# fuxiao0719/PanopticNeRF

Hardware: AMD Instinct MI355X
Metric: Msamples/sec (coarse+fine), KITTI-360 1408x376 (higher is better)
Workload: dtype bf16

## Files before the change

panopticnerf_amd/csrc/pnr_composite.hip:

```cpp
#include "pnr_composite_dev.h"

struct CompositeArgs {
    const float* raw; int64_t stride_s, stride_c;
    const float* z; const float* rays; const float* noise;
    const int32_t* label_sem; const int32_t* label_inst;
    int64_t R; int N, C, K, sem_mode, white_bkgd;
    float *rgb, *depth, *acc, *weights, *sem, *inst, *fix_sem, *fix_inst;
    int use_hist;
};

#ifndef CMP_GRID_PER_CU
#define CMP_GRID_PER_CU 8
#endif
#ifndef CMP_UB
#define CMP_UB 8
#endif

__device__ __forceinline__ float dot4(const f4& w, const f4& v)
{
    return fmaf(w.v[3], v.v[3], fmaf(w.v[2], v.v[2], fmaf(w.v[1], v.v[1], w.v[0] * v.v[0])));
}

template <bool CH_MAJOR, int SUB, bool SOFTMAX, class... Rng>
__global__ __launch_bounds__(256) void k_composite(CompositeArgs a, const Rng... rng)
{
    constexpr bool RNG = sizeof...(Rng) > 0;
    extern __shared__ __attribute__((aligned(16))) uint32_t s_hist[];
    RayLanes<SUB, 1> rl(a.R);
    const int wave = threadIdx.x >> 6;
    const int N = a.N, q = rl.q;
    const int CK = a.C + a.K;
    const int nq = 3 + CK;
    uint32_t* hist = s_hist + ((size_t)wave * rl.RPW + rl.g) * CK;
    PnrRngKey key;
    if constexpr (RNG) key = pnr_rng_key(rng...);

    const int64_t first = ((int64_t)blockIdx.x * blockDim.x + threadIdx.x) >> 6;
    const int64_t step = ((int64_t)gridDim.x * blockDim.x) >> 6;
    for (int64_t grp = first; grp < rl.n_groups; grp += step) {
        rl.at(grp, a.R, N);
        const int64_t ray = rl.ray, s0 = rl.s0;
        const bool active = rl.act[0];
        const bool writer = active && q == 0;

        const f4 zz = ld4(a.z + s0, active);
        f4 sg = load4<CH_MAJOR>(a.raw, a.stride_s, a.stride_c, s0, 3, active);
        f4 nxt[CMP_UB];
#pragma unroll
        for (int j = 0; j < CMP_UB; ++j) nxt[j] = load4<CH_MAJOR>(a.raw, a.stride_s, a.stride_c, s0, j < 3 ? j : j + 1, active && j < nq);
        add_sigma_noise4<RNG>(sg.v, active, key, (uint32_t)ray, (uint32_t)q, a.noise, a.noise + s0);
        const float dn = ray_dir_norm(a.rays, rl.rayc);
        const float znext = __shfl_down(zz.v[0], 1, 64);
        f4 alpha, Tl, w;
        float P = alpha_chain<4>(zz.v, znext, sg.v, rl.i0, N, dn, alpha.v, Tl.v);
        if (!active) P = 1.0f;
        const float excl = scan_excl_shfl<SUB>(P, q);
#pragma unroll
        for (int k = 0; k < 4; ++k) w.v[k] = active ? (alpha.v[k] * Tl.v[k]) * excl : 0.0f;
        if (a.weights) st4(a.weights + s0, w.v, active);
        const float accv = group_sum<SUB>((w.v[0] + w.v[1]) + (w.v[2] + w.v[3]));
        const float depv = group_sum<SUB>(dot4(w, zz));
        if (writer) {
            if (a.depth) a.depth[ray] = depv;
            if (a.acc) a.acc[ray] = accv;
        }

        const bool want_fs = a.fix_sem && a.label_sem && a.C, want_fi = a.fix_inst && a.label_inst && a.K;
        if (want_fs || want_fi) {
            int ls[4], li[4];
            ld4_labels(a.label_sem + s0, active && want_fs, ls);
            ld4_labels(a.label_inst + s0, active && want_fi, li);
            if (a.use_hist) {
                hist_zero<SUB>(hist, q, CK);
#pragma unroll
                for (int k = 0; k < 4; ++k) hist_add(hist, w.v[k], want_fs, ls[k], a.C, want_fi, li[k], a.K);
                if (rl.valid) hist_store<SUB>(hist, q, ray, want_fs, a.fix_sem, a.C, want_fi, a.fix_inst, a.K);
            } else {
                for (int c = 0; c < CK; ++c) {
                    const bool is_s = c < a.C;
                    if ((is_s && !want_fs) || (!is_s && !want_fi)) continue;
                    const int cc = is_s ? c : c - a.C;
                    float p = 0.0f;
#pragma unroll
                    for (int k = 0; k < 4; ++k) p += ((is_s ? ls[k] : li[k]) == cc) ? w.v[k] : 0.0f;
                    const float r = group_sum<SUB>(p);
                    if (writer) (is_s ? a.fix_sem : a.fix_inst)[ray * (is_s ? a.C : a.K) + cc] = r;
                }
            }
        }

        f4 mx_s, den_s, mx_i, den_i;
        if constexpr (SOFTMAX) {
            auto field_stats = [&](int nch, int ch0, f4& mx, f4& den) {
#pragma unroll
                for (int k = 0; k < 4; ++k) { mx.v[k] = -INFINITY; den.v[k] = 0.0f; }
                for (int c = 0; c < nch; ++c) {
                    const f4 v = load4<CH_MAJOR>(a.raw, a.stride_s, a.stride_c, s0, ch0 + c, active);
#pragma unroll
                    for (int k = 0; k < 4; ++k) lse_step(mx.v[k], den.v[k], v.v[k]);
                }
            };
            field_stats(a.C, 4, mx_s, den_s);
            field_stats(a.K, 4 + a.C, mx_i, den_i);
        }

#pragma unroll 1
        for (int q0 = 0; q0 < nq; q0 += CMP_UB) {
            float r[CMP_UB];
            const bool more = q0 + CMP_UB < nq;
#pragma unroll
            for (int j = 0; j < CMP_UB; ++j) {
                const int qq = q0 + j;
                f4 v = nxt[j];
                if (qq < 3) {
#pragma unroll
                    for (int k = 0; k < 4; ++k) v.v[k] = sigmoid_of(v.v[k]);
                } else if constexpr (SOFTMAX) {
                    const bool fs = (qq - 3) < a.C;
#pragma unroll
                    for (int k = 0; k < 4; ++k) v.v[k] = softmax_of(v.v[k], fs ? mx_s.v[k] : mx_i.v[k], fs ? den_s.v[k] : den_i.v[k]);
                }
                r[j] = dot4(w, v);
                const int q2 = qq + CMP_UB;
                if (more) nxt[j] = load4<CH_MAJOR>(a.raw, a.stride_s, a.stride_c, s0, q2 + 1, active && q2 < nq);
            }
            group_sum_batch<SUB, CMP_UB>(r);
            if (writer) store_rows<CMP_UB>(a, ray, q0, nq, r, accv);
        }
    }
}

#ifndef CMP2_UB
#define CMP2_UB 8
#endif

template <int L, int M4, bool SOFTMAX, class... Rng>
__global__ __launch_bounds__(256) void k_composite2(CompositeArgs a, const Rng... rng)
{
    constexpr bool RNG = sizeof...(Rng) > 0;
    extern __shared__ __attribute__((aligned(16))) uint32_t s_hist[];
    constexpr int M = 4 * M4;
    RayLanes<L, M4> rl(a.R);
    const int wave = threadIdx.x >> 6;
    const int N = a.N, q = rl.q, i0 = rl.i0;
    const int CK = a.C + a.K;
    const int nq = 3 + CK;
    uint32_t* hist = s_hist + ((size_t)wave * rl.RPW + rl.g) * CK;
    const int64_t sc = a.stride_c;
    PnrRngKey key;
    if constexpr (RNG) key = pnr_rng_key(rng...);

    const int64_t first = ((int64_t)blockIdx.x * blockDim.x + threadIdx.x) >> 6;
    const int64_t step = ((int64_t)gridDim.x * blockDim.x) >> 6;
    for (int64_t grp = first; grp < rl.n_groups; grp += step) {
        rl.at(grp, a.R, N);
        const int64_t ray = rl.ray, s0 = rl.s0;
        const bool (&act)[M4] = rl.act;
        const bool writer = rl.valid && q == 0;

        float zz[M], w[M];
        ld_row<M4>(a.z + s0, act, zz);
        ld_row<M4>(a.raw + 3 * sc + s0, act, w);
        float nxt[CMP2_UB][M];
#pragma unroll
        for (int j = 0; j < CMP2_UB; ++j) {
            if (j < nq) ld_row<M4>(a.raw + (int64_t)(j < 3 ? j : j + 1) * sc + s0, act, nxt[j]);
        }
#pragma unroll
        for (int j = 0; j < M4; ++j)
            add_sigma_noise4<RNG>(w + 4 * j, act[j], key, (uint32_t)ray, (uint32_t)((i0 >> 2) + j), a.noise, a.noise + s0 + 4 * j);
        const float dn = ray_dir_norm(a.rays, rl.rayc);
        const float znext = dpp_or<0x101>(zz[0], 0.0f);
        float alpha[M], Tl[M];
        float P = alpha_chain<M>(zz, znext, w, i0, N, dn, alpha, Tl);
        if (!act[0]) P = 1.0f;
        const float excl = scan_excl_dpp<L>(P, q);
        float accp = 0.0f, depp = 0.0f;
#pragma unroll
        for (int k = 0; k < M; ++k) {
            w[k] = act[k >> 2] ? (alpha[k] * Tl[k]) * excl : 0.0f;
            accp += w[k];
            depp = fmaf(w[k], zz[k], depp);
        }
        if (a.weights) {
#pragma unroll
            for (int j = 0; j < M4; ++j) st4(a.weights + s0 + 4 * j, w + 4 * j, act[j]);
        }
        const float accv = group_sum<L>(accp);
        const float depv = group_sum<L>(depp);
        if (writer) {
            if (a.depth) a.depth[ray] = depv;
            if (a.acc) a.acc[ray] = accv;
        }

        const bool want_fs = a.fix_sem && a.label_sem && a.C, want_fi = a.fix_inst && a.label_inst && a.K;
        if (want_fs || want_fi) {
            hist_zero<L>(hist, q, CK);
#pragma unroll
            for (int j = 0; j < M4; ++j) {
                int ls[4], li[4];
                ld4_labels(a.label_sem + s0 + 4 * j, act[j] && want_fs, ls);
                ld4_labels(a.label_inst + s0 + 4 * j, act[j] && want_fi, li);
#pragma unroll
                for (int k = 0; k < 4; ++k) hist_add(hist, w[4 * j + k], want_fs, ls[k], a.C, want_fi, li[k], a.K);
            }
            if (rl.valid) hist_store<L>(hist, q, ray, want_fs, a.fix_sem, a.C, want_fi, a.fix_inst, a.K);
        }

        float mx_s[SOFTMAX ? M : 1], den_s[SOFTMAX ? M : 1], mx_i[SOFTMAX ? M : 1], den_i[SOFTMAX ? M : 1];
        if constexpr (SOFTMAX) {
            auto field_stats = [&](int nch, int ch0, float (&mx)[M], float (&den)[M]) {
#pragma unroll
                for (int k = 0; k < M; ++k) { mx[k] = -INFINITY; den[k] = 0.0f; }
                for (int c = 0; c < nch; ++c) {
                    float v[M];
                    ld_row<M4>(a.raw + (int64_t)(ch0 + c) * sc + s0, act, v);
#pragma unroll
                    for (int k = 0; k < M; ++k) lse_step(mx[k], den[k], v[k]);
                }
            };
            field_stats(a.C, 4, mx_s, den_s);
            field_stats(a.K, 4 + a.C, mx_i, den_i);
        }

#pragma unroll 1
        for (int q0 = 0; q0 < nq; q0 += CMP2_UB) {
            float r[CMP2_UB];
#pragma unroll
            for (int j = 0; j < CMP2_UB; ++j) {
                const int qq = q0 + j;
                float acc = 0.0f;
#pragma unroll
                for (int k = 0; k < M; ++k) {
                    float v = nxt[j][k];
                    if (qq < 3) v = sigmoid_of(v);
                    else if constexpr (SOFTMAX) {
                        const bool fs = (qq - 3) < a.C;
                        v = softmax_of(v, fs ? mx_s[k] : mx_i[k], fs ? den_s[k] : den_i[k]);
                    }
                    acc = fmaf(w[k], v, acc);
                }
                r[j] = acc;
                const int q2 = qq + CMP2_UB;
                if (q2 < nq) ld_row<M4>(a.raw + (int64_t)(q2 + 1) * sc + s0, act, nxt[j]);
            }
            group_sum_batch<L, CMP2_UB>(r);
            if (writer) store_rows<CMP2_UB>(a, ray, q0, nq, r, accv);
        }
    }
}

static int composite_impl(const float* raw, int64_t raw_stride_s, int64_t raw_stride_c, const float* z, const float* rays,
                          const float* noise, const PnrRngDev* rng, const int32_t* label_sem, const int32_t* label_inst, int64_t n_rays,
                          int n_samples, int n_sem, int n_inst, int sem_mode, int white_bkgd, float* rgb, float* depth, float* acc,
                          float* weights, float* sem, float* inst, float* fix_sem, float* fix_inst, void* stream)
{
    PNR_REQUIRE(n_rays <= 0 || (raw && z && rays), "pnr_composite: null pointer");
    PNR_REQUIRE(n_samples >= 4 && n_samples <= 256 && (n_samples % 4) == 0,
                "pnr_composite: n_samples=%d must be a multiple of 4 in [4,256]", n_samples);
    PNR_REQUIRE(n_sem >= 0 && n_inst >= 0 && (sem_mode == 0 || sem_mode == 1), "pnr_composite: bad field sizes");
    PNR_REQUIRE((((uintptr_t)z) & 15) == 0, "pnr_composite: z must be 16-byte aligned");
    PNR_REQUIRE(!weights || (((uintptr_t)weights) & 15) == 0, "pnr_composite: weights must be 16-byte aligned");
    PNR_REQUIRE((((uintptr_t)noise) & 15) == 0 && (((uintptr_t)label_sem) & 15) == 0 && (((uintptr_t)label_inst) & 15) == 0,
                "pnr_composite: noise / label arrays must be 16-byte aligned");
    if (n_rays <= 0) return PNR_OK;
    CompositeArgs a;
    a.raw = raw; a.stride_s = raw_stride_s; a.stride_c = raw_stride_c; a.z = z; a.rays = rays; a.noise = noise;
    a.label_sem = label_sem; a.label_inst = label_inst; a.R = n_rays; a.N = n_samples; a.C = n_sem; a.K = n_inst;
    a.sem_mode = sem_mode; a.white_bkgd = white_bkgd; a.rgb = rgb; a.depth = depth; a.acc = acc; a.weights = weights;
    a.sem = sem; a.inst = inst; a.fix_sem = fix_sem; a.fix_inst = fix_inst;
    const bool want_fix = (fix_sem && label_sem && n_sem) || (fix_inst && label_inst && n_inst);
    const bool ch_major = raw_stride_s == 1 && (raw_stride_c % 4) == 0 && (((uintptr_t)raw) & 15) == 0;
    hipStream_t st = (hipStream_t)stream;
    auto hist_bytes = [&](int rpw) { return (size_t)4 * rpw * (n_sem + n_inst) * sizeof(uint32_t); };
    auto grid_for = [&](int rpw) { return pnr_grid_cap(((n_rays + rpw - 1) / rpw + 3) / 4, CMP_GRID_PER_CU); };
    if (ch_major && n_samples > 32 && n_samples <= 64 && (!want_fix || hist_bytes(8) <= 48 * 1024)) {
        a.use_hist = want_fix ? 1 : 0;
        const size_t lds = want_fix ? hist_bytes(8) : 0;
        composite_dispatch<8>(8, true, sem_mode, rng, [&](auto L, auto, auto SM, const auto&... r) {
            hipLaunchKernelGGL((k_composite2<decltype(L)::value, 2, decltype(SM)::value, std::decay_t<decltype(r)>...>), dim3(grid_for(8)), dim3(256),
                               lds, st, a, r...);
        });
        PNR_CHECK_LAUNCH("pnr_composite");
        return PNR_OK;
    }
    int sub = 1;
    while (sub < n_samples / 4) sub <<= 1;
    const int rpw = 64 / sub;
    a.use_hist = (want_fix && hist_bytes(rpw) <= 48 * 1024) ? 1 : 0;
    const size_t lds = a.use_hist ? hist_bytes(rpw) : 0;
    composite_dispatch<1, 2, 4, 8, 16, 32, 64>(sub, ch_major, sem_mode, rng, [&](auto S, auto CH, auto SM, const auto&... r) {
        hipLaunchKernelGGL((k_composite<decltype(CH)::value, decltype(S)::value, decltype(SM)::value, std::decay_t<decltype(r)>...>),
                           dim3(grid_for(rpw)), dim3(256), lds, st, a, r...);
    });
    PNR_CHECK_LAUNCH("pnr_composite");
    return PNR_OK;
}

PNR_EXPORT int pnr_composite(const float* raw, int64_t raw_stride_s, int64_t raw_stride_c, const float* z,
                             const float* rays, const float* noise, const int32_t* label_sem,
                             const int32_t* label_inst, int64_t n_rays, int n_samples, int n_sem, int n_inst,
                             int sem_mode, int white_bkgd, float* rgb, float* depth, float* acc, float* weights,
                             float* sem, float* inst, float* fix_sem, float* fix_inst, void* stream)
{
    return composite_impl(raw, raw_stride_s, raw_stride_c, z, rays, noise, nullptr, label_sem, label_inst, n_rays, n_samples, n_sem, n_inst,
                          sem_mode, white_bkgd, rgb, depth, acc, weights, sem, inst, fix_sem, fix_inst, stream);
}

PNR_EXPORT int pnr_composite_rng(const float* raw, int64_t raw_stride_s, int64_t raw_stride_c, const float* z, const float* rays,
                                 const pnr_rng* noise_host, const int32_t* label_sem, const int32_t* label_inst, int64_t n_rays,
                                 int n_samples, int n_sem, int n_inst, int sem_mode, int white_bkgd, float* rgb, float* depth, float* acc,
                                 float* weights, float* sem, float* inst, float* fix_sem, float* fix_inst, void* stream)
{
    PnrRngDev rng;
    const int rc = pnr_rng_check(noise_host, n_rays < 0 ? 0 : n_rays, "pnr_composite_rng", &rng);
    if (rc) return rc;
    PNR_REQUIRE(n_rays <= 0 || (raw_stride_s == 1 && (raw_stride_c % 4) == 0 && (((uintptr_t)raw) & 15) == 0),
                "pnr_composite_rng: channel-major, 16-byte aligned raw images only");
    return composite_impl(raw, raw_stride_s, raw_stride_c, z, rays, nullptr, &rng, label_sem, label_inst, n_rays, n_samples, n_sem, n_inst,
                          sem_mode, white_bkgd, rgb, depth, acc, weights, sem, inst, fix_sem, fix_inst, stream);
}

struct CombineArgs {
    const float* rec; int rec_floats; const float4* ps; const float* z; const int32_t* lab_s; const int32_t* lab_i;
    int64_t R; int N, C, K, white_bkgd;
    float *rgb, *depth, *acc, *weights, *sem, *inst, *fix_sem, *fix_inst;
};

template <bool LOGITS>
__global__ __launch_bounds__(256) void k_composite_combine(CombineArgs a)
{
    __shared__ uint32_t hist_all[4][128];
    const int lane = threadIdx.x & 63, wv = threadIdx.x >> 6;
    const int64_t ray = ((int64_t)blockIdx.x * blockDim.x + threadIdx.x) >> 6;
    if (ray >= a.R) return;
    const int N = a.N, T = N >> 5, RF = a.rec_floats, C = a.C, K = a.K, CK = C + K;
    const float* __restrict__ rec = a.rec + ray * T * RF;
    const float4* __restrict__ ps = a.ps + ray * N;
    const float* __restrict__ zr = a.z + ray * N;
    const bool want_s = a.lab_s && a.fix_sem && C, want_i = a.lab_i && a.fix_inst && K;
    const int32_t* __restrict__ lsr = want_s ? a.lab_s + ray * N : nullptr;
    const int32_t* __restrict__ lir = want_i ? a.lab_i + ray * N : nullptr;
    float q[8];
#pragma unroll
    for (int k = 0; k < 8; ++k) q[k] = k < T ? rec[k * RF] : 1.0f;
    float4 pv[4];
    float zv[4];
    int lsv[4], liv[4];
#pragma unroll
    for (int j = 0; j < 4; ++j) {
        const int i = lane + 64 * j;
        const bool in = i < N;
        pv[j] = in ? ps[i] : float4{0.0f, 0.0f, 0.0f, 0.0f};
        zv[j] = in ? zr[i] : 0.0f;
        lsv[j] = (in && want_s) ? lsr[i] : -1;
        liv[j] = (in && want_i) ? lir[i] : -1;
    }
    float lg[2][8];
#pragma unroll
    for (int h = 0; h < 2; ++h)
#pragma unroll
        for (int k = 0; k < 8; ++k) lg[h][k] = (LOGITS && k < T && lane + 64 * h < CK) ? rec[k * RF + PNR_FUSE_REC_LOGITS + lane + 64 * h] : 0.0f;
    float Tk[8];
    float t = 1.0f;
#pragma unroll
    for (int k = 0; k < 8; ++k) {
        Tk[k] = t;
        if (k < T) t *= q[k];
    }
    uint32_t* hist = hist_all[wv];
    if (want_s || want_i) hist_zero<64>(hist, lane, CK);
    float r5[5] = {0.0f, 0.0f, 0.0f, 0.0f, 0.0f};
#pragma unroll
    for (int j = 0; j < 4; ++j) {
        const int i = lane + 64 * j;
        if (i < N) {
            const float4 p = pv[j];
            float tk = Tk[0];
#pragma unroll
            for (int k = 1; k < 8; ++k) tk = (i >> 5) == k ? Tk[k] : tk;
            const float w = tk * p.x;
            r5[0] += w;
            r5[1] = fmaf(w, zv[j], r5[1]);
            r5[2] = fmaf(w, sigmoid_of(p.y), r5[2]);
            r5[3] = fmaf(w, sigmoid_of(p.z), r5[3]);
            r5[4] = fmaf(w, sigmoid_of(p.w), r5[4]);
            if (a.weights) a.weights[ray * N + i] = w;
            if (want_s || want_i) hist_add(hist, w, want_s, lsv[j], C, want_i, liv[j], K);
        }
    }
    group_sum_batch<64, 5>(r5);
    if (lane == 0) {
        if (a.acc) a.acc[ray] = r5[0];
        if (a.depth) a.depth[ray] = r5[1];
    }
    if (lane < 3 && a.rgb) {
        const float v = lane == 0 ? r5[2] : lane == 1 ? r5[3] : r5[4];
        a.rgb[ray * 3 + lane] = a.white_bkgd ? v + (1.0f - r5[0]) : v;
    }
#pragma unroll
    for (int h = 0; h < 2; ++h) {
        const int c = lane + 64 * h;
        if (c >= CK) continue;
        if constexpr (LOGITS) {
            float v = 0.0f;
#pragma unroll
            for (int k = 0; k < 8; ++k) if (k < T) v = fmaf(Tk[k], lg[h][k], v);
            if (c < C) { if (a.sem) a.sem[ray * C + c] = v; }
            else if (a.inst) a.inst[ray * K + (c - C)] = v;
        }
        if (c < C) { if (want_s) a.fix_sem[ray * C + c] = hist_read(hist, c); }
        else if (want_i) a.fix_inst[ray * K + (c - C)] = hist_read(hist, c);
    }
}

int pnr_composite_combine_launch(const float* rec, int rec_floats, bool logit_sums, const float4* ps, const float* z,
                                 const int32_t* label_sem, const int32_t* label_inst, int64_t R, int N, int C, int K, int white_bkgd,
                                 float* rgb, float* depth, float* acc, float* weights, float* sem, float* inst, float* fix_sem,
                                 float* fix_inst, hipStream_t st)
{
    CombineArgs a;
    a.rec = rec; a.rec_floats = rec_floats; a.ps = ps; a.z = z; a.lab_s = label_sem; a.lab_i = label_inst;
    a.R = R; a.N = N; a.C = C; a.K = K; a.white_bkgd = white_bkgd;
    a.rgb = rgb; a.depth = depth; a.acc = acc; a.weights = weights; a.sem = sem; a.inst = inst; a.fix_sem = fix_sem; a.fix_inst = fix_inst;
    const int64_t blocks = (R + 3) / 4;
    if (logit_sums) hipLaunchKernelGGL(k_composite_combine<true>, dim3((unsigned)blocks), dim3(256), 0, st, a);
    else hipLaunchKernelGGL(k_composite_combine<false>, dim3((unsigned)blocks), dim3(256), 0, st, a);
    PNR_CHECK_LAUNCH("pnr_mlp_forward_composite (combine)");
    return PNR_OK;
}
```

panopticnerf_amd/csrc/pnr_sampling.hip:

```cpp
#include "pnr_common.h"
#include "pnr_philox.h"
#include "pnr_sampling_dev.h"
#include <stdlib.h>
#include <string.h>

template <class... Rng>
__global__ __launch_bounds__(256) void k_stratified(const float* __restrict__ rays, int64_t R, int N,
                                                     int lindisp, const float* __restrict__ t_rand,
                                                     float* __restrict__ z_out, const Rng... rng)
{
    constexpr bool RNG = sizeof...(Rng) > 0;
    PnrRngKey key;
    if constexpr (RNG) key = pnr_rng_key(rng...);
    const int64_t total = R * N;
    for (int64_t s = (int64_t)blockIdx.x * blockDim.x + threadIdx.x; s < total;
         s += (int64_t)gridDim.x * blockDim.x) {
        const int64_t r = s / N;
        const int i = (int)(s - r * N);
        if constexpr (RNG) {
            const float t = pnr_rng_uniform_at(key, (uint32_t)r, i);
            z_out[s] = strat_sample(rays[r * 8 + 6], rays[r * 8 + 7], i, N, lindisp, &t);
        } else {
            z_out[s] = strat_sample(rays[r * 8 + 6], rays[r * 8 + 7], i, N, lindisp, t_rand ? t_rand + s : nullptr);
        }
    }
}

__global__ __launch_bounds__(256) void k_points(const float* __restrict__ rays, const float* __restrict__ z,
                                                 int64_t R, int N, float* __restrict__ pts)
{
    const int64_t total = R * N * 3;
    for (int64_t e = (int64_t)blockIdx.x * blockDim.x + threadIdx.x; e < total;
         e += (int64_t)gridDim.x * blockDim.x) {
        const int64_t s = e / 3;
        const int a = (int)(e - s * 3);
        const int64_t r = s / N;
        const float m = rays[r * 8 + 3 + a] * z[s];
        pts[e] = rays[r * 8 + a] + m;
    }
}

__global__ __launch_bounds__(256) void k_embed(const float* __restrict__ x, int64_t n, int L,
                                                float* __restrict__ out)
{
    const int E = 3 + 6 * L;
    const int64_t total = n * E;
    for (int64_t e = (int64_t)blockIdx.x * blockDim.x + threadIdx.x; e < total;
         e += (int64_t)gridDim.x * blockDim.x) {
        const int64_t s = e / E;
        const int c = (int)(e - s * E);
        float v;
        if (c < 3) {
            v = x[s * 3 + c];
        } else {
            const int k = (c - 3) / 6, j = (c - 3) - 6 * k;
            const int a = j % 3;
            const float arg = x[s * 3 + a] * ldexpf(1.0f, k);
            v = (j < 3) ? sinf(arg) : cosf(arg);
        }
        out[e] = v;
    }
}

struct PdfLabelArgs {
    const float* hit_t; const int32_t* hit_box; const int32_t* hit_count; int max_hits; const int32_t* box_ids;
    int32_t* label_sem; int32_t* label_inst;
};
#define PDF_MAXC 256
#define PDF_MAXT 512
template <int MAXC, int MAXT, class... Rng>
__device__ __forceinline__ void sample_pdf_body(const float* __restrict__ z, const float* __restrict__ weights,
                                                    const float* __restrict__ u, int64_t R, int Nc, int Nf,
                                                    float* __restrict__ zs_out, int32_t* __restrict__ inds_out,
                                                    float* __restrict__ zfine_out, const PdfLabelArgs lab, const Rng&... rng)
{
    constexpr bool RNG = sizeof...(Rng) > 0;
    PnrRngKey key;
    if constexpr (RNG) key = pnr_rng_key(rng...);
    __shared__ float s_z[MAXC], s_w[MAXC], s_pdf[MAXC], s_cdf[MAXC], s_bins[MAXC];
    __shared__ float s_sort[MAXT], s_out[MAXT];
    __shared__ float s_total, s_part[32];
    const int lane = threadIdx.x;
    const int nb = Nc - 1, nw = Nc - 2, Nt = Nc + Nf;
    const int P = pdf_padded(Nt);
    auto labels = [&](int64_t r, const float* sorted) {
        if (!lab.label_sem) return;
        const int mh = lab.max_hits;
        const int cnt = lab.hit_count[r] < mh ? lab.hit_count[r] : mh;
        for (int i = lane; i < Nt; i += 64) {
            const int best = label_hit(sorted[i], cnt, [&](int h, float& ti, float& to) {
                ti = lab.hit_t[(r * mh + h) * 2];
                to = lab.hit_t[(r * mh + h) * 2 + 1];
            });
            int ls, li;
            hit_ids(best, lab.hit_box + r * mh + best, lab.box_ids, &ls, &li);
            lab.label_sem[r * Nt + i] = ls;
            lab.label_inst[r * Nt + i] = li;
        }
    };
    for (int64_t r = blockIdx.x; r < R; r += gridDim.x) {
        for (int i = lane; i < Nc; i += 64) {
            s_z[i] = z[r * Nc + i];
            s_w[i] = weights[r * Nc + i];
        }
        __syncthreads();
        for (int k = lane; k < nb; k += 64) s_bins[k] = 0.5f * (s_z[k + 1] + s_z[k]);
        const float total = pdf_torch_total(s_w, nw, s_part, &s_total, lane);
        for (int j = lane; j < nw; j += 64) s_pdf[j] = (s_w[j + 1] + 1e-5f) / total;
        __syncthreads();
        pdf_cdf(lane < nw ? s_pdf[lane < nw ? lane : 0] : 0.0f, nw, nw <= 64, s_pdf, s_cdf, lane);
        for (int i = lane; i < Nf; i += 64) {
            float uu;
            if constexpr (RNG) uu = pnr_rng_uniform_at(key, (uint32_t)r, i);
            else uu = u ? u[r * Nf + i] : pnr_linspace01(i, Nf);
            int lo = 0, hi = nb;
            while (lo < hi) {
                const int mid = (lo + hi) >> 1;
                if (s_cdf[mid] <= uu) lo = mid + 1; else hi = mid;
            }
            const float zs = pdf_invert(uu, lo, nb, s_cdf, s_bins);
            if (zs_out) zs_out[r * Nf + i] = zs;
            if (inds_out) inds_out[r * Nf + i] = lo;
            s_sort[Nc + i] = zs;
        }
        if (zfine_out) {
            __syncthreads();
            bool asc = true;
            for (int i = lane; i + 1 < Nf; i += 64) asc = asc && (s_sort[Nc + i] <= s_sort[Nc + i + 1]);
            for (int i = lane; i + 1 < Nc; i += 64) asc = asc && (s_z[i] <= s_z[i + 1]);
            if (__all(asc)) {
                for (int i = lane; i < Nc; i += 64) {
                    const float v = s_z[i];
                    int lo = 0, hi = Nf;
                    while (lo < hi) { const int mid = (lo + hi) >> 1; if (s_sort[Nc + mid] < v) lo = mid + 1; else hi = mid; }
                    s_out[i + lo] = v;
                }
                for (int j = lane; j < Nf; j += 64) {
                    const float v = s_sort[Nc + j];
                    int lo = 0, hi = Nc;
                    while (lo < hi) { const int mid = (lo + hi) >> 1; if (s_z[mid] <= v) lo = mid + 1; else hi = mid; }
                    s_out[j + lo] = v;
                }
                __syncthreads();
                for (int i = lane; i < Nt; i += 64) zfine_out[r * Nt + i] = s_out[i];
                labels(r, s_out);
                __syncthreads();
                continue;
            }
            for (int i = lane; i < Nc; i += 64) s_sort[i] = s_z[i];
            for (int i = Nt + lane; i < P; i += 64) s_sort[i] = INFINITY;
            __syncthreads();
            pdf_bitonic(s_sort, P, lane);
            for (int i = lane; i < Nt; i += 64) zfine_out[r * Nt + i] = s_sort[i];
            labels(r, s_sort);
        }
        __syncthreads();
    }
}

__device__ __noinline__ void pdf_bitonic_fallback(float* s_sort, const float* s_z, const float* s_zs, int Nc, int Nf, int P, int lane)
{
    const int Nt = Nc + Nf;
    for (int i = lane; i < Nc; i += 64) s_sort[i] = s_z[i];
    for (int i = lane; i < Nf; i += 64) s_sort[Nc + i] = s_zs[i];
    for (int i = Nt + lane; i < P; i += 64) s_sort[i] = INFINITY;
    __syncthreads();
    pdf_bitonic(s_sort, P, lane);
}

#ifndef PDF_DET_WPE
#define PDF_DET_WPE 8
#endif
#if PDF_DET_WPE
__attribute__((amdgpu_waves_per_eu(PDF_DET_WPE, PDF_DET_WPE)))
#endif
__global__ __launch_bounds__(64) void k_sample_pdf_det(const float* __restrict__ z, const float* __restrict__ weights, int64_t R, int Nc,
                                                        int Nf, float* __restrict__ zfine_out, const PdfLabelArgs lab)
{
    __shared__ float s_z[64], s_w[64], s_pdf[64], s_cdf[64], s_bins[64];
    __shared__ float s_zs[192], s_out[256];
    __shared__ float s_total, s_part[32];
    const int lane = threadIdx.x;
    const int nb = Nc - 1, nw = Nc - 2, Nt = Nc + Nf;
    int topc = 1, topf = 1;
    while (topc * 2 <= Nc) topc *= 2;
    while (topf * 2 <= Nf) topf *= 2;
    const int mh = lab.max_hits;
    for (int64_t r = blockIdx.x; r < R; r += gridDim.x) {
        const float* __restrict__ zr = z + r * Nc;
        const float* __restrict__ wr = weights + r * Nc;
        const float zl = lane < Nc ? zr[lane] : 0.0f, wl = lane < Nc ? wr[lane] : 0.0f;
        int cnt = 0, h_ls = -1, h_li = -1;
        float h_ti = 0.0f, h_to = 0.0f;
        if (lab.label_sem) {
            const int c0 = lab.hit_count[r];
            cnt = c0 < mh ? c0 : mh;
            if (lane < cnt) {
                const float2 t2 = *reinterpret_cast<const float2*>(lab.hit_t + (r * mh + lane) * 2);
                h_ti = t2.x; h_to = t2.y;
                hit_ids(lane, lab.hit_box + r * mh + lane, lab.box_ids, &h_ls, &h_li);
            }
        }
        s_z[lane] = zl;
        s_w[lane] = wl;
        const float zn = __shfl_down(zl, 1, 64), wn = __shfl_down(wl, 1, 64);
        s_bins[lane] = 0.5f * (zn + zl);
        __syncthreads();
        const float total = pdf_torch_total(s_w, nw, s_part, &s_total, lane);
        const float pl = lane < nw ? (wn + 1e-5f) / total : 0.0f;
        s_pdf[lane] = pl;
        pdf_cdf(pl, nw, true, s_pdf, s_cdf, lane);
        bool asc = lane + 1 >= Nc || zl <= zn;
        for (int i = lane; i < Nf; i += 64) {
            const float uu = pnr_linspace01(i, Nf);
            int pos = 0;
            for (int st = topc; st >= 1; st >>= 1) {
                const int p = pos + st, q = p <= nb ? p : nb;
                pos = (p <= nb && s_cdf[q - 1] <= uu) ? p : pos;
            }
            s_zs[i] = pdf_invert(uu, pos, nb, s_cdf, s_bins);
        }
        __syncthreads();
        for (int i = lane; i + 1 < Nf; i += 64) asc = asc && (s_zs[i] <= s_zs[i + 1]);
        if (__all(asc)) {
            if (lane < Nc) {
                int pos = 0;
                for (int st = topf; st >= 1; st >>= 1) {
                    const int p = pos + st, q = p <= Nf ? p : Nf;
                    pos = (p <= Nf && s_zs[q - 1] < zl) ? p : pos;
                }
                s_out[lane + pos] = zl;
            }
            for (int j = lane; j < Nf; j += 64) {
                const float v = s_zs[j];
                int pos = 0;
                for (int st = topc; st >= 1; st >>= 1) {
                    const int p = pos + st, q = p <= Nc ? p : Nc;
                    pos = (p <= Nc && s_z[q - 1] <= v) ? p : pos;
                }
                s_out[j + pos] = v;
            }
            __syncthreads();
        } else {
            pdf_bitonic_fallback(s_out, s_z, s_zs, Nc, Nf, pdf_padded(Nt), lane);
        }
        float* __restrict__ zo = zfine_out + r * Nt;
        for (int i0 = 0; i0 < Nt; i0 += 256) {
            float zz[4];
            int best[4], ls[4], li[4];
            float bt[4];
#pragma unroll
            for (int k = 0; k < 4; ++k) {
                const int i = i0 + lane + 64 * k;
                zz[k] = i < Nt ? s_out[i < Nt ? i : 0] : 0.0f;
                best[k] = -1; ls[k] = -1; li[k] = -1; bt[k] = 0.0f;
                if (i < Nt) zo[i] = zz[k];
            }
            if (lab.label_sem) {
                for (int h = 0; h < cnt; ++h) {
                    const float ti = __int_as_float(__builtin_amdgcn_readlane(__float_as_int(h_ti), h));
                    const float to = __int_as_float(__builtin_amdgcn_readlane(__float_as_int(h_to), h));
                    const int hs = __builtin_amdgcn_readlane(h_ls, h), hi2 = __builtin_amdgcn_readlane(h_li, h);
#pragma unroll
                    for (int k = 0; k < 4; ++k) {
                        const bool take = ti <= zz[k] && zz[k] <= to && (best[k] < 0 || ti < bt[k]);
                        best[k] = take ? h : best[k];
                        bt[k] = take ? ti : bt[k];
                        ls[k] = take ? hs : ls[k];
                        li[k] = take ? hi2 : li[k];
                    }
                }
#pragma unroll
                for (int k = 0; k < 4; ++k) {
                    const int i = i0 + lane + 64 * k;
                    if (i < Nt) {
                        lab.label_sem[r * Nt + i] = ls[k];
                        lab.label_inst[r * Nt + i] = li[k];
                    }
                }
            }
        }
        __syncthreads();
    }
}

template <int MAXC, int MAXT, class... Rng>
__global__ __launch_bounds__(64) __attribute__((amdgpu_waves_per_eu(MAXC <= 64 ? 8 : 1, 8)))
void k_sample_pdf(const float* __restrict__ z, const float* __restrict__ weights, const float* __restrict__ u, int64_t R, int Nc, int Nf,
                  float* __restrict__ zs_out, int32_t* __restrict__ inds_out, float* __restrict__ zfine_out, const PdfLabelArgs lab,
                  const Rng... rng)
{
    sample_pdf_body<MAXC, MAXT>(z, weights, u, R, Nc, Nf, zs_out, inds_out, zfine_out, lab, rng...);
}

__global__ __launch_bounds__(256) void k_bbox_hits(const float* __restrict__ rays, int64_t R,
                                                    const float* __restrict__ box, int M, int max_hits,
                                                    float* __restrict__ hit_t, int32_t* __restrict__ hit_box,
                                                    int32_t* __restrict__ hit_count)
{
    for (int64_t r = (int64_t)blockIdx.x * blockDim.x + threadIdx.x; r < R;
         r += (int64_t)gridDim.x * blockDim.x) {
        const RayRec ry = ray_load(rays, r);
        const auto list = hit_rows(hit_t, hit_box, r, max_hits);
        hit_init(list, max_hits);
        int cnt = 0;
        for (int m = 0; m < M; ++m) {
            float tmin, tmax;
            slab_interval(box + m * 15, ry, &tmin, &tmax);
            if (tmin <= tmax) hit_insert(list, cnt, max_hits, tmin, tmax, m);
        }
        hit_count[r] = cnt;
    }
}

#define SETUP_MAXH 8
struct RaySetupArgs {
    const float* rays; int64_t R; const float* box; int M; int max_hits; const int32_t* box_ids;
    int N, lindisp, hull; const float* t_rand;
    float* hit_t; int32_t* hit_box; int32_t* hit_count; float* z; int32_t* label_sem; int32_t* label_inst;
};
template <class... Rng>
__global__ __launch_bounds__(256) void k_ray_setup(const RaySetupArgs a, const Rng... rng)
{
    constexpr bool RNG = sizeof...(Rng) > 0;
    __shared__ float2 s_t[SETUP_MAXH][64];
    __shared__ float s_nr[64], s_fr[64];
    __shared__ int s_hb[SETUP_MAXH][64], s_cnt[64];
    const int tid = threadIdx.x, lane = tid & 63, wv = tid >> 6;
    const int mh = a.max_hits, N = a.N;
    PnrRngKey key;
    if constexpr (RNG) key = pnr_rng_key(rng...);
    for (int64_t base = (int64_t)blockIdx.x * 64; base < a.R; base += (int64_t)gridDim.x * 64) {
        const int64_t r = base + tid;
        if (tid < 64 && r < a.R) {
            const float4 ra = *reinterpret_cast<const float4*>(a.rays + r * 8), rb = *reinterpret_cast<const float4*>(a.rays + r * 8 + 4);
            const float o0 = ra.x, o1 = ra.y, o2 = ra.z, d0 = ra.w, d1 = rb.x, d2 = rb.y;
            float nr = rb.z, fr = rb.w;
            for (int h = 0; h < SETUP_MAXH; ++h) { s_hb[h][tid] = -1; s_t[h][tid] = make_float2(0.0f, 0.0f); }
            int cnt = 0;
            for (int m = 0; m < a.M; ++m) {
                const float* b = a.box + m * 15;
                const float p0 = o0 - b[0], p1 = o1 - b[1], p2 = o2 - b[2];
                float tmin = nr, tmax = fr;
#pragma unroll
                for (int x = 0; x < 3; ++x) {
                    const float r0 = b[3 + 3 * x], r1 = b[4 + 3 * x], r2 = b[5 + 3 * x];
                    const float ol = (r0 * p0 + r1 * p1) + r2 * p2;
                    const float dl = (r0 * d0 + r1 * d1) + r2 * d2;
                    const float inv = 1.0f / dl;
                    const float e = b[12 + x];
                    const float t1 = (-e - ol) * inv, t2 = (e - ol) * inv;
                    tmin = fmaxf(tmin, fminf(t1, t2));
                    tmax = fminf(tmax, fmaxf(t1, t2));
                }
                if (tmin <= tmax) {
                    const int n = cnt < mh ? cnt : mh;
                    int pos = n;
                    while (pos > 0 && s_t[pos - 1][tid].x > tmin) --pos;
                    if (pos < mh) {
                        for (int k = (n < mh ? n : mh - 1); k > pos; --k) {
                            s_t[k][tid] = s_t[k - 1][tid];
                            s_hb[k][tid] = s_hb[k - 1][tid];
                        }
                        s_t[pos][tid] = make_float2(tmin, tmax);
                        s_hb[pos][tid] = m;
                    }
                    ++cnt;
                }
            }
            a.hit_count[r] = cnt;
            const int kept = cnt < mh ? cnt : mh;
            for (int h = 0; h < mh; ++h) {
                *reinterpret_cast<float2*>(a.hit_t + (r * mh + h) * 2) = s_t[h][tid];
                a.hit_box[r * mh + h] = s_hb[h][tid];
            }
            if (a.hull && kept > 0) {
                float lo = s_t[0][tid].x, hi = s_t[0][tid].y;
                for (int h = 1; h < kept; ++h) {
                    lo = fminf(lo, s_t[h][tid].x);
                    hi = fmaxf(hi, s_t[h][tid].y);
                }
                nr = lo; fr = hi;
            }
            s_nr[tid] = nr; s_fr[tid] = fr; s_cnt[tid] = kept;
        }
        __syncthreads();
        constexpr int RU = 2;
        for (int rr = wv * 16; rr < wv * 16 + 16; rr += RU) {
            if (base + rr >= a.R) break;
            float nr[RU], fr[RU];
            int cnt[RU], hb[RU][SETUP_MAXH];
            float2 iv[RU][SETUP_MAXH];
#pragma unroll
            for (int u = 0; u < RU; ++u) {
                const int t = rr + u;
                auto uni = [](float v) { return __int_as_float(__builtin_amdgcn_readfirstlane(__float_as_int(v))); };
                nr[u] = uni(s_nr[t]); fr[u] = uni(s_fr[t]);
                cnt[u] = __builtin_amdgcn_readfirstlane(s_cnt[t]);
#pragma unroll
                for (int h = 0; h < SETUP_MAXH; ++h) {
                    const float2 v = s_t[h][t];
                    iv[u][h] = make_float2(uni(v.x), uni(v.y));
                    hb[u][h] = __builtin_amdgcn_readfirstlane(s_hb[h][t]);
                }
            }
#pragma unroll
            for (int u = 0; u < RU; ++u) {
                const int64_t ray = base + rr + u;
                if (ray >= a.R) break;
                for (int i = lane; i < N; i += 64) {
                    const int64_t s = ray * N + i;
                    float zz;
                    if constexpr (RNG) {
                        const float t = pnr_rng_uniform_at(key, (uint32_t)ray, i);
                        zz = strat_sample(nr[u], fr[u], i, N, a.lindisp, &t);
                    } else {
                        zz = strat_sample(nr[u], fr[u], i, N, a.lindisp, a.t_rand ? a.t_rand + s : nullptr);
                    }
                    a.z[s] = zz;
                    if (a.label_sem) {
                        int best = -1, m = -1;
                        float bt = 0.0f;
#pragma unroll
                        for (int h = 0; h < SETUP_MAXH; ++h) {
                            if (h >= cnt[u]) break;
                            const float ti = iv[u][h].x, to = iv[u][h].y;
                            if (ti <= zz && zz <= to && (best < 0 || ti < bt)) { best = h; bt = ti; m = hb[u][h]; }
                        }
                        int ls = -1, li = -1;
                        if (best >= 0) {
                            ls = a.box_ids[m * 2];
                            li = a.box_ids[m * 2 + 1];
                        }
                        a.label_sem[s] = ls;
                        a.label_inst[s] = li;
                    }
                }
            }
        }
        __syncthreads();
    }
}

__global__ __launch_bounds__(256) void k_sample_labels(const float* __restrict__ z, int64_t R, int N,
                                                        const float* __restrict__ hit_t,
                                                        const int32_t* __restrict__ hit_box,
                                                        const int32_t* __restrict__ hit_count, int max_hits,
                                                        const int32_t* __restrict__ box_ids,
                                                        int32_t* __restrict__ label_sem,
                                                        int32_t* __restrict__ label_inst)
{
    const int64_t total = R * N;
    for (int64_t s = (int64_t)blockIdx.x * blockDim.x + threadIdx.x; s < total;
         s += (int64_t)gridDim.x * blockDim.x) {
        const int64_t r = s / N;
        const float zz = z[s];
        const int cnt = hit_count[r] < max_hits ? hit_count[r] : max_hits;
        const int best = label_hit(zz, cnt, [&](int h, float& ti, float& to) {
            ti = hit_t[(r * max_hits + h) * 2];
            to = hit_t[(r * max_hits + h) * 2 + 1];
        });
        int ls = -1, li = -1;
        if (best >= 0) {
            const int m = hit_box[r * max_hits + best];
            ls = box_ids[m * 2];
            li = box_ids[m * 2 + 1];
        }
        label_sem[s] = ls;
        label_inst[s] = li;
    }
}

PNR_EXPORT int pnr_stratified(const float* rays, int64_t n_rays, int n_samples, int lindisp,
                              const float* t_rand, float* z_out, void* stream)
{
    PNR_REQUIRE(n_rays >= 0 && n_samples >= 1, "pnr_stratified: bad size R=%lld N=%d", (long long)n_rays, n_samples);
    if (n_rays == 0) return PNR_OK;
    PNR_REQUIRE(rays && z_out, "pnr_stratified: null pointer");
    const int64_t total = n_rays * n_samples;
    hipLaunchKernelGGL(k_stratified<>, dim3(pnr_grid_cap((total + 255) / 256)), dim3(256), 0, (hipStream_t)stream,
                       rays, n_rays, n_samples, lindisp, t_rand, z_out);
    PNR_CHECK_LAUNCH("pnr_stratified");
    return PNR_OK;
}

PNR_EXPORT int pnr_stratified_rng(const float* rays, int64_t n_rays, int n_samples, int lindisp, const pnr_rng* rng_host,
                                  float* z_out, void* stream)
{
    PnrRngDev rng;
    const int rc = pnr_rng_check(rng_host, n_rays, "pnr_stratified_rng", &rng);
    if (rc) return rc;
    PNR_REQUIRE(n_rays >= 0 && n_samples >= 1 && n_samples <= (1 << 26), "pnr_stratified_rng: bad size R=%lld N=%d", (long long)n_rays,
                n_samples);
    if (n_rays == 0) return PNR_OK;
    PNR_REQUIRE(rays && z_out, "pnr_stratified_rng: null pointer");
    const int64_t total = n_rays * n_samples;
    hipLaunchKernelGGL(k_stratified<PnrRngDev>, dim3(pnr_grid_cap((total + 255) / 256)), dim3(256), 0, (hipStream_t)stream,
                       rays, n_rays, n_samples, lindisp, (const float*)nullptr, z_out, rng);
    PNR_CHECK_LAUNCH("pnr_stratified_rng");
    return PNR_OK;
}

PNR_EXPORT int pnr_points(const float* rays, const float* z, int64_t n_rays, int n_samples, float* pts_out,
                          void* stream)
{
    PNR_REQUIRE(n_rays >= 0 && n_samples >= 1, "pnr_points: bad size");
    if (n_rays == 0) return PNR_OK;
    PNR_REQUIRE(rays && z && pts_out, "pnr_points: null pointer");
    const int64_t total = n_rays * n_samples * 3;
    hipLaunchKernelGGL(k_points, dim3(pnr_grid_cap((total + 255) / 256)), dim3(256), 0, (hipStream_t)stream,
                       rays, z, n_rays, n_samples, pts_out);
    PNR_CHECK_LAUNCH("pnr_points");
    return PNR_OK;
}

PNR_EXPORT int pnr_embed(const float* x, int64_t n, int L, float* out, void* stream)
{
    PNR_REQUIRE(n >= 0 && L >= 0 && L <= 16, "pnr_embed: bad size n=%lld L=%d", (long long)n, L);
    if (n == 0) return PNR_OK;
    PNR_REQUIRE(x && out, "pnr_embed: null pointer");
    const int64_t total = n * (3 + 6 * L);
    hipLaunchKernelGGL(k_embed, dim3(pnr_grid_cap((total + 255) / 256)), dim3(256), 0, (hipStream_t)stream,
                       x, n, L, out);
    PNR_CHECK_LAUNCH("pnr_embed");
    return PNR_OK;
}

static void launch_sample_pdf(const float* z, const float* weights, const float* u, const PnrRngDev* rng, int64_t n_rays, int n_coarse,
                              int n_fine, float* z_samples, int32_t* inds, float* z_fine, const PdfLabelArgs& lab, hipStream_t st)
{
    const dim3 grid(pnr_grid_cap(n_rays, 32)), block(64);
    const bool small = n_coarse <= 64 && pdf_padded(n_coarse + n_fine) <= 256;
    auto go = [&](auto kernel, auto... r) {
        hipLaunchKernelGGL(kernel, grid, block, 0, st, z, weights, u, n_rays, n_coarse, n_fine, z_samples, inds, z_fine, lab, r...);
    };
    if (!rng && !u && !z_samples && !inds && z_fine && small && n_fine <= 192 && lab.max_hits <= 64 && !getenv("PNR_SAMPLE_PDF_GENERAL"))
        hipLaunchKernelGGL(k_sample_pdf_det, grid, block, 0, st, z, weights, n_rays, n_coarse, n_fine, z_fine, lab);
    else if (rng)
        go(small ? k_sample_pdf<64, 256, PnrRngDev> : k_sample_pdf<PDF_MAXC, PDF_MAXT, PnrRngDev>, *rng);
    else
        go(small ? k_sample_pdf<64, 256> : k_sample_pdf<PDF_MAXC, PDF_MAXT>);
}

static int sample_pdf_impl(const char* name, const float* z, const float* weights, const float* u, bool with_rng, const pnr_rng* rng_host,
                           int64_t n_rays, int n_coarse, int n_fine, float* z_samples, int32_t* inds, float* z_fine,
                           const PdfLabelArgs* labels, void* stream)
{
    PnrRngDev rng;
    if (with_rng) {
        const int rc = pnr_rng_check(rng_host, n_rays < 0 ? 0 : n_rays, name, &rng);
        if (rc) return rc;
    }
    PNR_REQUIRE(n_rays <= 0 || (z && weights && (!labels || z_fine)), "%s: null pointer", name);
    PNR_REQUIRE(!labels || n_rays <= 0 || (labels->hit_t && labels->hit_box && labels->hit_count && labels->box_ids && labels->label_sem &&
                                           labels->label_inst), "%s: null pointer", name);
    PNR_REQUIRE(n_coarse >= 3 && n_coarse <= PDF_MAXC, "%s: n_coarse=%d outside [3,%d]", name, n_coarse, PDF_MAXC);
    PNR_REQUIRE(n_fine >= 1 && n_coarse + n_fine <= PDF_MAXT, "%s: n_coarse+n_fine=%d > %d", name, n_coarse + n_fine, PDF_MAXT);
    PNR_REQUIRE(!labels || labels->max_hits >= 1, "%s: bad max_hits", name);
    if (n_rays <= 0) return PNR_OK;
    launch_sample_pdf(z, weights, u, with_rng ? &rng : nullptr, n_rays, n_coarse, n_fine, z_samples, inds, z_fine,
                      labels ? *labels : PdfLabelArgs{}, (hipStream_t)stream);
    PNR_CHECK_LAUNCH(name);
    return PNR_OK;
}

PNR_EXPORT int pnr_sample_pdf(const float* z, const float* weights, const float* u, int64_t n_rays, int n_coarse,
                              int n_fine, float* z_samples, int32_t* inds, float* z_fine, void* stream)
{
    return sample_pdf_impl("pnr_sample_pdf", z, weights, u, false, nullptr, n_rays, n_coarse, n_fine, z_samples, inds, z_fine, nullptr, stream);
}

PNR_EXPORT int pnr_sample_pdf_rng(const float* z, const float* weights, const pnr_rng* rng_host, int64_t n_rays, int n_coarse,
                                  int n_fine, float* z_samples, int32_t* inds, float* z_fine, void* stream)
{
    return sample_pdf_impl("pnr_sample_pdf_rng", z, weights, nullptr, true, rng_host, n_rays, n_coarse, n_fine, z_samples, inds, z_fine, nullptr,
                           stream);
}

PNR_EXPORT int pnr_sample_pdf_labels(const float* z, const float* weights, const float* u, int64_t n_rays, int n_coarse, int n_fine,
                                     float* z_fine, const float* hit_t, const int32_t* hit_box, const int32_t* hit_count,
                                     int max_hits, const int32_t* box_ids, int32_t* label_sem, int32_t* label_inst, void* stream)
{
    const PdfLabelArgs lab{hit_t, hit_box, hit_count, max_hits, box_ids, label_sem, label_inst};
    return sample_pdf_impl("pnr_sample_pdf_labels", z, weights, u, false, nullptr, n_rays, n_coarse, n_fine, nullptr, nullptr, z_fine, &lab, stream);
}

PNR_EXPORT int pnr_sample_pdf_labels_rng(const float* z, const float* weights, const pnr_rng* rng_host, int64_t n_rays, int n_coarse,
                                         int n_fine, float* z_fine, const float* hit_t, const int32_t* hit_box, const int32_t* hit_count,
                                         int max_hits, const int32_t* box_ids, int32_t* label_sem, int32_t* label_inst, void* stream)
{
    const PdfLabelArgs lab{hit_t, hit_box, hit_count, max_hits, box_ids, label_sem, label_inst};
    return sample_pdf_impl("pnr_sample_pdf_labels_rng", z, weights, nullptr, true, rng_host, n_rays, n_coarse, n_fine, nullptr, nullptr, z_fine,
                           &lab, stream);
}

static int ray_setup_impl(const float* rays, int64_t n_rays, const float* box, int n_box, int max_hits, const int32_t* box_ids,
                          int n_samples, int lindisp, const float* t_rand, const PnrRngDev* rng, int hull, float* hit_t, int32_t* hit_box,
                          int32_t* hit_count, float* z_out, int32_t* label_sem, int32_t* label_inst, void* stream);

PNR_EXPORT int pnr_ray_setup(const float* rays, int64_t n_rays, const float* box, int n_box, int max_hits, const int32_t* box_ids,
                             int n_samples, int lindisp, const float* t_rand, int hull, float* hit_t, int32_t* hit_box,
                             int32_t* hit_count, float* z_out, int32_t* label_sem, int32_t* label_inst, void* stream)
{
    return ray_setup_impl(rays, n_rays, box, n_box, max_hits, box_ids, n_samples, lindisp, t_rand, nullptr, hull, hit_t, hit_box, hit_count,
                          z_out, label_sem, label_inst, stream);
}

PNR_EXPORT int pnr_ray_setup_rng(const float* rays, int64_t n_rays, const float* box, int n_box, int max_hits, const int32_t* box_ids,
                                 int n_samples, int lindisp, const pnr_rng* rng_host, int hull, float* hit_t, int32_t* hit_box,
                                 int32_t* hit_count, float* z_out, int32_t* label_sem, int32_t* label_inst, void* stream)
{
    PnrRngDev rng;
    const int rc = pnr_rng_check(rng_host, n_rays < 0 ? 0 : n_rays, "pnr_ray_setup_rng", &rng);
    if (rc) return rc;
    PNR_REQUIRE(n_samples <= (1 << 26), "pnr_ray_setup_rng: n_samples=%d > 2^26", n_samples);
    return ray_setup_impl(rays, n_rays, box, n_box, max_hits, box_ids, n_samples, lindisp, nullptr, &rng, hull, hit_t, hit_box, hit_count,
                          z_out, label_sem, label_inst, stream);
}

static int ray_setup_impl(const float* rays, int64_t n_rays, const float* box, int n_box, int max_hits, const int32_t* box_ids,
                          int n_samples, int lindisp, const float* t_rand, const PnrRngDev* rng, int hull, float* hit_t, int32_t* hit_box,
                          int32_t* hit_count, float* z_out, int32_t* label_sem, int32_t* label_inst, void* stream)
{
    PNR_REQUIRE(n_rays >= 0 && n_samples >= 1, "pnr_ray_setup: bad size R=%lld N=%d", (long long)n_rays, n_samples);
    PNR_REQUIRE(max_hits >= 1 && max_hits <= SETUP_MAXH, "pnr_ray_setup: max_hits=%d outside [1,%d] (use the separate entry points)",
                max_hits, SETUP_MAXH);
    PNR_REQUIRE(n_box >= 0 && (n_box == 0 || box), "pnr_ray_setup: bad box table");
    if (n_rays == 0) return PNR_OK;
    PNR_REQUIRE(rays && hit_t && hit_box && hit_count && z_out, "pnr_ray_setup: null pointer");
    PNR_REQUIRE((label_sem != nullptr) == (label_inst != nullptr) && (!label_sem || box_ids || n_box == 0),
                "pnr_ray_setup: labels need both outputs and box_ids");
    PNR_REQUIRE((((uintptr_t)rays) & 15) == 0 && (((uintptr_t)hit_t) & 7) == 0, "pnr_ray_setup: rays must be 16-byte aligned");
    RaySetupArgs a;
    a.rays = rays; a.R = n_rays; a.box = box; a.M = n_box; a.max_hits = max_hits; a.box_ids = box_ids;
    a.N = n_samples; a.lindisp = lindisp; a.hull = hull; a.t_rand = t_rand;
    a.hit_t = hit_t; a.hit_box = hit_box; a.hit_count = hit_count; a.z = z_out; a.label_sem = label_sem; a.label_inst = label_inst;
    if (rng)
        hipLaunchKernelGGL(k_ray_setup<PnrRngDev>, dim3(pnr_grid_cap((n_rays + 63) / 64)), dim3(256), 0, (hipStream_t)stream, a, *rng);
    else
        hipLaunchKernelGGL(k_ray_setup<>, dim3(pnr_grid_cap((n_rays + 63) / 64)), dim3(256), 0, (hipStream_t)stream, a);
    PNR_CHECK_LAUNCH("pnr_ray_setup");
    return PNR_OK;
}

PNR_EXPORT int pnr_bbox_hits(const float* rays, int64_t n_rays, const float* box, int n_box, int max_hits,
                             float* hit_t, int32_t* hit_box, int32_t* hit_count, void* stream)
{
    PNR_REQUIRE(n_rays <= 0 || (rays && hit_t && hit_box && hit_count), "pnr_bbox_hits: null pointer");
    PNR_REQUIRE(n_box >= 0 && (n_box == 0 || box), "pnr_bbox_hits: bad box table");
    PNR_REQUIRE(max_hits >= 1 && max_hits <= 64, "pnr_bbox_hits: max_hits=%d outside [1,64]", max_hits);
    if (n_rays <= 0) return PNR_OK;
    hipLaunchKernelGGL(k_bbox_hits, dim3(pnr_grid_cap((n_rays + 255) / 256)), dim3(256), 0, (hipStream_t)stream,
                       rays, n_rays, box, n_box, max_hits, hit_t, hit_box, hit_count);
    PNR_CHECK_LAUNCH("pnr_bbox_hits");
    return PNR_OK;
}

PNR_EXPORT int pnr_sample_labels(const float* z, int64_t n_rays, int n_samples, const float* hit_t,
                                 const int32_t* hit_box, const int32_t* hit_count, int max_hits,
                                 const int32_t* box_ids, int32_t* label_sem, int32_t* label_inst, void* stream)
{
    PNR_REQUIRE(n_rays <= 0 || (z && hit_t && hit_box && hit_count && box_ids && label_sem && label_inst),
                "pnr_sample_labels: null pointer");
    PNR_REQUIRE(n_samples >= 1 && max_hits >= 1, "pnr_sample_labels: bad size");
    if (n_rays <= 0) return PNR_OK;
    const int64_t total = n_rays * n_samples;
    hipLaunchKernelGGL(k_sample_labels, dim3(pnr_grid_cap((total + 255) / 256)), dim3(256), 0,
                       (hipStream_t)stream, z, n_rays, n_samples, hit_t, hit_box, hit_count, max_hits, box_ids,
                       label_sem, label_inst);
    PNR_CHECK_LAUNCH("pnr_sample_labels");
    return PNR_OK;
}

__global__ __launch_bounds__(256) void k_restrict_rays(const float* __restrict__ rays, int64_t R, const float* __restrict__ hit_t,
                                                        const int32_t* __restrict__ hit_count, int max_hits, float* __restrict__ out)
{
    for (int64_t r = (int64_t)blockIdx.x * blockDim.x + threadIdx.x; r < R; r += (int64_t)gridDim.x * blockDim.x) {
        const float4 a = *reinterpret_cast<const float4*>(rays + r * 8);
        float4 b = *reinterpret_cast<const float4*>(rays + r * 8 + 4);
        const int cnt = hit_count[r] < max_hits ? hit_count[r] : max_hits;
        if (cnt > 0) hit_hull(HitRows<const float, const int32_t>{hit_t + r * max_hits * 2, nullptr}, cnt, &b.z, &b.w);
        *reinterpret_cast<float4*>(out + r * 8) = a;
        *reinterpret_cast<float4*>(out + r * 8 + 4) = b;
    }
}

PNR_EXPORT int pnr_restrict_rays(const float* rays, int64_t n_rays, const float* hit_t, const int32_t* hit_count, int max_hits,
                                 float* rays_out, void* stream)
{
    PNR_REQUIRE(n_rays >= 0 && max_hits >= 1, "pnr_restrict_rays: bad size");
    if (n_rays == 0) return PNR_OK;
    PNR_REQUIRE(rays && hit_t && hit_count && rays_out, "pnr_restrict_rays: null pointer");
    PNR_REQUIRE(((((uintptr_t)rays) | ((uintptr_t)rays_out)) & 15) == 0, "pnr_restrict_rays: ray records must be 16-byte aligned");
    hipLaunchKernelGGL(k_restrict_rays, dim3(pnr_grid_cap((n_rays + 255) / 256)), dim3(256), 0, (hipStream_t)stream, rays, n_rays,
                       hit_t, hit_count, max_hits, rays_out);
    PNR_CHECK_LAUNCH("pnr_restrict_rays");
    return PNR_OK;
}
```

Measured before the change: 1170.

## Replace per-sample CDF binary search with scatter-count scan; specialize combine for small N

In the deterministic PDF sampler, each CDF edge now computes its rank among the uniform linspace points, atomically increments a shared histogram, and a DPP wave prefix-scan turns the counts into bin indices. This replaces the per-fine-sample binary search over the CDF. The change adds an extra barrier and LDS atomics, and it relies on the rank test exactly matching the old comparison semantics. Separately, the composite combine kernel is templated on the sample-tile counts, so coarse passes with N<=64 use small register arrays.

```diff
diff --git a/panopticnerf_amd/csrc/pnr_composite.hip b/panopticnerf_amd/csrc/pnr_composite.hip
--- a/panopticnerf_amd/csrc/pnr_composite.hip
+++ b/panopticnerf_amd/csrc/pnr_composite.hip
@@ -327,7 +327,7 @@
     float *rgb, *depth, *acc, *weights, *sem, *inst, *fix_sem, *fix_inst;
 };
 
-template <bool LOGITS>
+template <bool LOGITS, int MT, int MJ>
 __global__ __launch_bounds__(256) void k_composite_combine(CombineArgs a)
 {
     __shared__ uint32_t hist_all[4][128];
@@ -341,14 +341,14 @@
     const bool want_s = a.lab_s && a.fix_sem && C, want_i = a.lab_i && a.fix_inst && K;
     const int32_t* __restrict__ lsr = want_s ? a.lab_s + ray * N : nullptr;
     const int32_t* __restrict__ lir = want_i ? a.lab_i + ray * N : nullptr;
-    float q[8];
-#pragma unroll
-    for (int k = 0; k < 8; ++k) q[k] = k < T ? rec[k * RF] : 1.0f;
-    float4 pv[4];
-    float zv[4];
-    int lsv[4], liv[4];
-#pragma unroll
-    for (int j = 0; j < 4; ++j) {
+    float q[MT];
+#pragma unroll
+    for (int k = 0; k < MT; ++k) q[k] = k < T ? rec[k * RF] : 1.0f;
+    float4 pv[MJ];
+    float zv[MJ];
+    int lsv[MJ], liv[MJ];
+#pragma unroll
+    for (int j = 0; j < MJ; ++j) {
         const int i = lane + 64 * j;
         const bool in = i < N;
         pv[j] = in ? ps[i] : float4{0.0f, 0.0f, 0.0f, 0.0f};
@@ -356,15 +356,15 @@
         lsv[j] = (in && want_s) ? lsr[i] : -1;
         liv[j] = (in && want_i) ? lir[i] : -1;
     }
-    float lg[2][8];
+    float lg[2][MT];
 #pragma unroll
     for (int h = 0; h < 2; ++h)
 #pragma unroll
-        for (int k = 0; k < 8; ++k) lg[h][k] = (LOGITS && k < T && lane + 64 * h < CK) ? rec[k * RF + PNR_FUSE_REC_LOGITS + lane + 64 * h] : 0.0f;
-    float Tk[8];
+        for (int k = 0; k < MT; ++k) lg[h][k] = (LOGITS && k < T && lane + 64 * h < CK) ? rec[k * RF + PNR_FUSE_REC_LOGITS + lane + 64 * h] : 0.0f;
+    float Tk[MT];
     float t = 1.0f;
 #pragma unroll
-    for (int k = 0; k < 8; ++k) {
+    for (int k = 0; k < MT; ++k) {
         Tk[k] = t;
         if (k < T) t *= q[k];
     }
@@ -372,13 +372,13 @@
     if (want_s || want_i) hist_zero<64>(hist, lane, CK);
     float r5[5] = {0.0f, 0.0f, 0.0f, 0.0f, 0.0f};
 #pragma unroll
-    for (int j = 0; j < 4; ++j) {
+    for (int j = 0; j < MJ; ++j) {
         const int i = lane + 64 * j;
         if (i < N) {
             const float4 p = pv[j];
             float tk = Tk[0];
 #pragma unroll
-            for (int k = 1; k < 8; ++k) tk = (i >> 5) == k ? Tk[k] : tk;
+            for (int k = 1; k < MT; ++k) tk = (i >> 5) == k ? Tk[k] : tk;
             const float w = tk * p.x;
             r5[0] += w;
             r5[1] = fmaf(w, zv[j], r5[1]);
@@ -405,7 +405,7 @@
         if constexpr (LOGITS) {
             float v = 0.0f;
 #pragma unroll
-            for (int k = 0; k < 8; ++k) if (k < T) v = fmaf(Tk[k], lg[h][k], v);
+            for (int k = 0; k < MT; ++k) if (k < T) v = fmaf(Tk[k], lg[h][k], v);
             if (c < C) { if (a.sem) a.sem[ray * C + c] = v; }
             else if (a.inst) a.inst[ray * K + (c - C)] = v;
         }
@@ -424,8 +424,9 @@
     a.R = R; a.N = N; a.C = C; a.K = K; a.white_bkgd = white_bkgd;
     a.rgb = rgb; a.depth = depth; a.acc = acc; a.weights = weights; a.sem = sem; a.inst = inst; a.fix_sem = fix_sem; a.fix_inst = fix_inst;
     const int64_t blocks = (R + 3) / 4;
-    if (logit_sums) hipLaunchKernelGGL(k_composite_combine<true>, dim3((unsigned)blocks), dim3(256), 0, st, a);
-    else hipLaunchKernelGGL(k_composite_combine<false>, dim3((unsigned)blocks), dim3(256), 0, st, a);
+    auto go = [&](auto kernel) { hipLaunchKernelGGL(kernel, dim3((unsigned)blocks), dim3(256), 0, st, a); };
+    if (N <= 64) go(logit_sums ? k_composite_combine<true, 2, 1> : k_composite_combine<false, 2, 1>);
+    else go(logit_sums ? k_composite_combine<true, 8, 4> : k_composite_combine<false, 8, 4>);
     PNR_CHECK_LAUNCH("pnr_mlp_forward_composite (combine)");
     return PNR_OK;
 }
diff --git a/panopticnerf_amd/csrc/pnr_sampling.hip b/panopticnerf_amd/csrc/pnr_sampling.hip
--- a/panopticnerf_amd/csrc/pnr_sampling.hip
+++ b/panopticnerf_amd/csrc/pnr_sampling.hip
@@ -168,6 +168,29 @@
     pdf_bitonic(s_sort, P, lane);
 }
 
+__device__ __forceinline__ int pdf_rank_in_u(float c, int Nf)
+{
+    const int e = (int)fminf(fmaxf(c * (float)(Nf - 1), 0.0f), (float)Nf);
+    int n = e - 1;
+#pragma unroll
+    for (int d = -1; d <= 1; ++d) {
+        const int j = e + d;
+        n += (j < 0 || (j < Nf && pnr_linspace01(j, Nf) < c)) ? 1 : 0;
+    }
+    return n;
+}
+
+__device__ __forceinline__ int wave_scan_add(int x)
+{
+    x += __builtin_amdgcn_update_dpp(0, x, 0x111, 0xF, 0xF, false);
+    x += __builtin_amdgcn_update_dpp(0, x, 0x112, 0xF, 0xF, false);
+    x += __builtin_amdgcn_update_dpp(0, x, 0x114, 0xF, 0xF, false);
+    x += __builtin_amdgcn_update_dpp(0, x, 0x118, 0xF, 0xF, false);
+    x += __builtin_amdgcn_update_dpp(0, x, 0x142, 0xA, 0xF, false);
+    x += __builtin_amdgcn_update_dpp(0, x, 0x143, 0xC, 0xF, false);
+    return x;
+}
+
 #ifndef PDF_DET_WPE
 #define PDF_DET_WPE 8
 #endif
@@ -180,11 +203,13 @@
     __shared__ float s_z[64], s_w[64], s_pdf[64], s_cdf[64], s_bins[64];
     __shared__ float s_zs[192], s_out[256];
     __shared__ float s_total, s_part[32];
+    __shared__ int s_cnt[192];
     const int lane = threadIdx.x;
     const int nb = Nc - 1, nw = Nc - 2, Nt = Nc + Nf;
     int topc = 1, topf = 1;
     while (topc * 2 <= Nc) topc *= 2;
     while (topf * 2 <= Nf) topf *= 2;
+    const int per = (Nf + 63) >> 6;
     const int mh = lab.max_hits;
     for (int64_t r = blockIdx.x; r < R; r += gridDim.x) {
         const float* __restrict__ zr = z + r * Nc;
@@ -205,20 +230,31 @@
         s_w[lane] = wl;
         const float zn = __shfl_down(zl, 1, 64), wn = __shfl_down(wl, 1, 64);
         s_bins[lane] = 0.5f * (zn + zl);
+        for (int i = lane; i < Nf; i += 64) s_cnt[i] = 0;
         __syncthreads();
         const float total = pdf_torch_total(s_w, nw, s_part, &s_total, lane);
         const float pl = lane < nw ? (wn + 1e-5f) / total : 0.0f;
         s_pdf[lane] = pl;
         pdf_cdf(pl, nw, true, s_pdf, s_cdf, lane);
         bool asc = lane + 1 >= Nc || zl <= zn;
-        for (int i = lane; i < Nf; i += 64) {
-            const float uu = pnr_linspace01(i, Nf);
-            int pos = 0;
-            for (int st = topc; st >= 1; st >>= 1) {
-                const int p = pos + st, q = p <= nb ? p : nb;
-                pos = (p <= nb && s_cdf[q - 1] <= uu) ? p : pos;
-            }
-            s_zs[i] = pdf_invert(uu, pos, nb, s_cdf, s_bins);
+        if (lane < nb) {
+            const int jk = pdf_rank_in_u(s_cdf[lane], Nf);
+            if (jk < Nf) atomicAdd(&s_cnt[jk], 1);
+        }
+        __syncthreads();
+        int cn[3], own = 0;
+#pragma unroll
+        for (int m = 0; m < 3; ++m) {
+            const int j = lane * per + m;
+            cn[m] = (m < per && j < Nf) ? s_cnt[j < Nf ? j : 0] : 0;
+            own += cn[m];
+        }
+        int inds = wave_scan_add(own) - own;
+#pragma unroll
+        for (int m = 0; m < 3; ++m) {
+            const int j = lane * per + m;
+            inds += cn[m];
+            if (m < per && j < Nf) s_zs[j] = pdf_invert(pnr_linspace01(j, Nf), inds, nb, s_cdf, s_bins);
         }
         __syncthreads();
         for (int i = lane; i + 1 < Nf; i += 64) asc = asc && (s_zs[i] <= s_zs[i + 1]);
```

After: 1173 (median of 6 runs). No clear change (+0.2%).
